# DeepMETv2/DeepMETv2

Measured on AMD Instinct MI355X. Metric: events/sec (4.5k PF cands, k=16), higher is better.
Workload: dtype f32

## Files before the change

deepmetv2_amd/build.py:

```python
from __future__ import annotations

import concurrent.futures as cf
import os
import shutil
import subprocess
import sys

PKG_DIR = os.path.dirname(os.path.abspath(__file__))
CSRC = os.path.join(PKG_DIR, "csrc")
OBJ_DIR = os.path.join(CSRC, "_obj")
LIB_PATH = os.path.join(PKG_DIR, "libdmet_hip.so")
SOURCES = ["knn.hip", "radius.hip", "edgeconv.hip", "edgemlp.hip", "misc.hip", "dense.hip", "encoder.hip", "norm.hip", "edgeconv_bwd.hip",
           "head.hip", "finalize.hip", "pool.hip",
           "edgemlp_f32.hip", "edgemlp_bf16.hip", "edgeconv_sum.hip", "gravnet.hip", "attention.hip", "fps.hip", "interpolate.hip",
           "pointnet.hip", "gat.hip", "segment.hip", "multi_aggr.hip", "weighted_sum.hip", "event_norm.hip", "select.hip"]
HEADERS = [os.path.join(CSRC, h) for h in ("common.h", "bn_affine.h", "knn_common.h", "knn_filter.h", "knn_key64.h", "knn_tile_schedule.h",
                                           "nls_body.h",
                                           "edgemlp_fused.h", "row_softmax.h")] + \
          [os.path.join(PKG_DIR, "..", "include", "dmet.h")]
ARCH = "gfx950"
CXXFLAGS = ["-O3", "-std=c++17", "-fPIC", f"--offload-arch={ARCH}", "-ffp-contract=off", "-Wall",
            "-Wno-unused-function", "-DNDEBUG"]


def _hipcc() -> str:
    exe = shutil.which("hipcc") or "/opt/rocm/bin/hipcc"
    if not os.path.exists(exe):
        raise RuntimeError("hipcc not found: cannot build libdmet_hip.so")
    return exe


def _stale(target: str, deps) -> bool:
    if not os.path.exists(target):
        return True
    t = os.path.getmtime(target)
    return any(os.path.getmtime(d) > t for d in deps if os.path.exists(d))


def _compile(src: str, force: bool) -> str:
    obj = os.path.join(OBJ_DIR, os.path.splitext(src)[0] + ".o")
    path = os.path.join(CSRC, src)
    if force or _stale(obj, [path] + HEADERS):
        cmd = [_hipcc()] + CXXFLAGS + ["-c", path, "-o", obj]
        subprocess.check_call(cmd)
    return obj


def build_hip(force: bool = False, verbose: bool = False) -> str:
    os.makedirs(OBJ_DIR, exist_ok=True)
    with cf.ThreadPoolExecutor(max_workers=min(4, len(SOURCES))) as ex:
        objs = list(ex.map(lambda s: _compile(s, force), SOURCES))
    if force or _stale(LIB_PATH, objs):
        cmd = [_hipcc(), "-shared", "-fPIC", f"--offload-arch={ARCH}", "-o", LIB_PATH] + objs
        if verbose:
            print(" ".join(cmd))
        subprocess.check_call(cmd)
    return LIB_PATH


if __name__ == "__main__":
    print(build_hip(force="--force" in sys.argv, verbose=True))
```

deepmetv2_amd/csrc/common.h:

```cpp
#pragma once
#include <hip/hip_runtime.h>
#include <stdint.h>
#include <stdio.h>
#include <stdlib.h>
#include <string.h>

#include <type_traits>

#include "../../include/dmet.h"

namespace dmet {

constexpr int kWave = 64;
constexpr int kNumXcd = 8;
constexpr float kKnnSentinel = 1e10f;

void set_error(const char *fmt, ...);
int hip_fail(hipError_t e, const char *what);

#define DMET_REQUIRE(cond, ...)                 \
    do {                                        \
        if (!(cond)) {                          \
            ::dmet::set_error(__VA_ARGS__);     \
            return -22;                         \
        }                                       \
    } while (0)

#define DMET_LAUNCH_CHECK(name)                                   \
    do {                                                          \
        hipError_t e__ = hipGetLastError();                       \
        if (e__ != hipSuccess) return ::dmet::hip_fail(e__, name); \
    } while (0)

static inline hipStream_t as_stream(dmet_stream_t s) { return reinterpret_cast<hipStream_t>(s); }

static inline bool env_is(const char *name, const char *value)
{
    const char *e = getenv(name);
    return e && strcmp(e, value) == 0;
}

static inline bool aligned16(const void *p) { return (reinterpret_cast<uintptr_t>(p) & 15u) == 0; }

__device__ __forceinline__ int find_event(const int64_t *__restrict__ ptr, int B, int64_t i)
{
    int lo = 0, hi = B;
    while (hi - lo > 1) {
        const int mid = (lo + hi) >> 1;
        if (ptr[mid] <= i) lo = mid; else hi = mid;
    }
    return lo;
}

__device__ __forceinline__ int xcd_swizzle(int bid, int nblk)
{
    const int q = nblk / kNumXcd, rm = nblk % kNumXcd;
    const int xcd = bid % kNumXcd, idx = bid / kNumXcd;
    const int base = (xcd < rm) ? xcd * (q + 1) : rm * (q + 1) + (xcd - rm) * q;
    return base + idx;
}

constexpr int kEcbPartialFloats = 2 * 1024 + 32;
constexpr int kEncPartialFloats = 3 * 1024 + 64;
constexpr int kHeadPartialFloats = 1024 + 64;
enum { kDeferEdgeConv = 0, kDeferEncoder = 1, kDeferHead = 2 };
struct DeferDesc {
    int kind;
    const float *partial;
    int64_t nparts;
    float *out[9];
};
bool defer_push(const DeferDesc &d);

__device__ __forceinline__ float wave_sum(float v)
{
#pragma unroll
    for (int off = 32; off > 0; off >>= 1) v += __shfl_xor(v, off, 64);
    return v;
}

template <int... Vs, typename F>
bool with_int(int v, F &&f)
{
    return ((v == Vs && (f(std::integral_constant<int, Vs>{}), true)) || ...);
}
template <typename F>
void with_flags(F &&f) { f(); }
template <typename F, typename... Rest>
void with_flags(F &&f, bool b, Rest... rest)
{
    if (b) with_flags([&](auto... c) { f(std::true_type{}, c...); }, rest...);
    else with_flags([&](auto... c) { f(std::false_type{}, c...); }, rest...);
}

}
```

deepmetv2_amd/csrc/encoder.hip:

```cpp
#include <stdlib.h>

#include "bn_affine.h"
#include "common.h"

namespace dmet {
namespace {

typedef float f32x16 __attribute__((ext_vector_type(16)));

#define ENC_PARAMS                                                                                                  \
    const float *__restrict__ Wc, const float *__restrict__ bc, const float *__restrict__ Wk,                      \
        const float *__restrict__ bk, const float *__restrict__ Wa, const float *__restrict__ ba,                  \
        const float *__restrict__ Echg, const float *__restrict__ Epdg, const float *__restrict__ Epv
#define ENC_ARGS Wc, bc, Wk, bk, Wa, ba, Echg, Epdg, Epv

__device__ __forceinline__ float elu(float z) { return z > 0.0f ? z : (__expf(z) - 1.0f); }

__device__ __forceinline__ void cat_indices(const int64_t *__restrict__ xcat, const float *__restrict__ row, int64_t i,
                                            int &ichg, int &ipdg, int &ipv)
{
    long long c = xcat ? xcat[i * 3 + 0] : (long long)row[8];
    const long long chg = xcat ? xcat[i * 3 + 1] : (long long)row[9];
    const long long pv = xcat ? xcat[i * 3 + 2] : (long long)row[10];
    c = c < 0 ? -c : c;
    const long long table[7] = {1, 2, 11, 13, 22, 130, 211};
#pragma unroll
    for (int t = 0; t < 7; ++t) c = (c == table[t]) ? (long long)t : c;
    ipdg = (int)min(max(c, 0ll), 6ll);
    ichg = (int)min(max(chg + 1, 0ll), 2ll);
    ipv = (int)min(max(pv, 0ll), 7ll);
}

__device__ __forceinline__ void encode_node(ENC_PARAMS, const float (&xc)[8], int ichg, int ipdg, int ipv,
                                            float (&cat24)[24], float (&z1)[16], float (&z2)[16], float (&joint)[32],
                                            float (&z3)[32])
{
#pragma unroll
    for (int e = 0; e < 8; ++e) {
        cat24[e] = Echg[ichg * 8 + e];
        cat24[8 + e] = Epdg[ipdg * 8 + e];
        cat24[16 + e] = Epv[ipv * 8 + e];
    }
#pragma unroll
    for (int o = 0; o < 16; ++o) {
        float a = bc[o];
#pragma unroll
        for (int f = 0; f < 8; ++f) a = __builtin_fmaf(Wc[o * 8 + f], xc[f], a);
        z1[o] = a;
        float b = bk[o];
#pragma unroll
        for (int f = 0; f < 24; ++f) b = __builtin_fmaf(Wk[o * 24 + f], cat24[f], b);
        z2[o] = b;
    }
#pragma unroll
    for (int o = 0; o < 16; ++o) { joint[o] = elu(z2[o]); joint[16 + o] = elu(z1[o]); }
#pragma unroll
    for (int o = 0; o < 32; ++o) {
        float a = ba[o];
#pragma unroll
        for (int f = 0; f < 32; ++f) a = __builtin_fmaf(Wa[o * 32 + f], joint[f], a);
        z3[o] = a;
    }
}

__global__ __launch_bounds__(256, 2) void encode_fwd_kernel(const float *__restrict__ x, int64_t x_stride,
                                                          const int64_t *__restrict__ xcat, int64_t N,
                                                          ENC_PARAMS, float *__restrict__ h)
{
    const int64_t i = (int64_t)blockIdx.x * blockDim.x + threadIdx.x;
    if (i >= N) return;
    const float *row = x + i * x_stride;
    float xc[8];
#pragma unroll
    for (int f = 0; f < 8; ++f) xc[f] = row[f];
    int ichg, ipdg, ipv;
    cat_indices(xcat, row, i, ichg, ipdg, ipv);
    float cat24[24], z1[16], z2[16], joint[32], z3[32];
    encode_node(ENC_ARGS, xc, ichg, ipdg, ipv, cat24, z1, z2, joint, z3);
    float4 *o = reinterpret_cast<float4 *>(h + i * 32);
#pragma unroll
    for (int c = 0; c < 8; ++c)
        o[c] = make_float4(elu(z3[4 * c]), elu(z3[4 * c + 1]), elu(z3[4 * c + 2]), elu(z3[4 * c + 3]));
}

__global__ __launch_bounds__(256) void encode_fwd_mfma_kernel(const float *__restrict__ x, int64_t x_stride,
                                                               const int64_t *__restrict__ xcat, int64_t N, ENC_PARAMS,
                                                               float *__restrict__ h)
{
    const int lane = threadIdx.x & 63, r = lane & 31, hh = lane >> 5;
    const int64_t wave = (int64_t)blockIdx.x * (blockDim.x >> 6) + __builtin_amdgcn_readfirstlane((int)(threadIdx.x >> 6));
    const int64_t nwaves = (int64_t)gridDim.x * (blockDim.x >> 6);
    const int64_t ntiles = (N + 31) / 32;
    float w12[16], w3[16], b12[16], b3[16];
#pragma unroll
    for (int s = 0; s < 16; ++s) {
        const int f = (s & 3) + 8 * (s >> 2) + 4 * hh;
        const float *src = r < 16 ? Wk + r * 24 + min(f, 23) : Wc + (r - 16) * 8 + max(f - 24, 0);
        const bool keep = r < 16 ? f < 24 : f >= 24;
        const float a = *src;
        w12[s] = keep ? a : 0.0f;
        w3[s] = Wa[r * 32 + f];
        const float *bsrc = f < 16 ? bk + f : bc + (f - 16);
        b12[s] = *bsrc;
        b3[s] = ba[f];
    }
    struct Raw { float c[4]; long long k0, k1, k2; };
    auto load_raw = [&](const int64_t tile, Raw &q) __attribute__((always_inline)) {
        const int64_t node = tile * 32 + r;
        const int64_t i = node < N ? node : N - 1;
        const float *row = x + i * x_stride;
#pragma unroll
        for (int u = 0; u < 4; ++u) q.c[u] = row[4 * hh + u];
        if (xcat) { q.k0 = xcat[i * 3 + 0]; q.k1 = xcat[i * 3 + 1]; q.k2 = xcat[i * 3 + 2]; }
        else { q.k0 = (long long)row[8]; q.k1 = (long long)row[9]; q.k2 = (long long)row[10]; }
    };
    auto load_tables = [&](const Raw &q, float (&in)[16]) __attribute__((always_inline)) {
        long long c = q.k0 < 0 ? -q.k0 : q.k0;
        const long long table[7] = {1, 2, 11, 13, 22, 130, 211};
#pragma unroll
        for (int t = 0; t < 7; ++t) c = (c == table[t]) ? (long long)t : c;
        const int ipdg = (int)min(max(c, 0ll), 6ll), ichg = (int)min(max(q.k1 + 1, 0ll), 2ll), ipv = (int)min(max(q.k2, 0ll), 7ll);
        const float4 e0 = *reinterpret_cast<const float4 *>(Echg + ichg * 8 + 4 * hh);
        const float4 e1 = *reinterpret_cast<const float4 *>(Epdg + ipdg * 8 + 4 * hh);
        const float4 e2 = *reinterpret_cast<const float4 *>(Epv + ipv * 8 + 4 * hh);
        in[0] = e0.x; in[1] = e0.y; in[2] = e0.z; in[3] = e0.w; in[4] = e1.x; in[5] = e1.y; in[6] = e1.z; in[7] = e1.w;
        in[8] = e2.x; in[9] = e2.y; in[10] = e2.z; in[11] = e2.w;
#pragma unroll
        for (int u = 0; u < 4; ++u) in[12 + u] = q.c[u];
    };
    Raw raw;
    float in[16], nxt[16];
    if (wave < ntiles) { load_raw(wave, raw); load_tables(raw, in); }
    if (wave + nwaves < ntiles) load_raw(wave + nwaves, raw);
    for (int64_t tile = wave; tile < ntiles; tile += nwaves) {
        const int64_t node = tile * 32 + r;
        if (tile + nwaves < ntiles) load_tables(raw, nxt);
        if (tile + 2 * nwaves < ntiles) load_raw(tile + 2 * nwaves, raw);
        f32x16 acc;
#pragma unroll
        for (int e = 0; e < 16; ++e) acc[e] = b12[e];
#pragma unroll
        for (int s = 0; s < 16; ++s) acc = __builtin_amdgcn_mfma_f32_32x32x2f32(w12[s], in[s], acc, 0, 0, 0);
        float joint[16];
#pragma unroll
        for (int e = 0; e < 16; ++e) joint[e] = elu(acc[e]);
#pragma unroll
        for (int e = 0; e < 16; ++e) acc[e] = b3[e];
#pragma unroll
        for (int s = 0; s < 16; ++s) acc = __builtin_amdgcn_mfma_f32_32x32x2f32(w3[s], joint[s], acc, 0, 0, 0);
        if (node < N) {
            float4 *o = reinterpret_cast<float4 *>(h + node * 32 + 4 * hh);
#pragma unroll
            for (int g = 0; g < 4; ++g)
                o[2 * g] = make_float4(elu(acc[4 * g]), elu(acc[4 * g + 1]), elu(acc[4 * g + 2]), elu(acc[4 * g + 3]));
        }
#pragma unroll
        for (int u = 0; u < 16; ++u) in[u] = nxt[u];
    }
}

constexpr int kEncTiles = 3;
constexpr int kEncBwdWaves = 4;
constexpr int kEncPartial = kEncTiles * 1024 + 64;

__device__ __forceinline__ void enc_wave_sync()
{
    __builtin_amdgcn_fence(__ATOMIC_RELEASE, "wavefront");
    __builtin_amdgcn_wave_barrier();
    __builtin_amdgcn_fence(__ATOMIC_ACQUIRE, "wavefront");
}

__device__ __forceinline__ void tile_mma(f32x16 &acc, const float *__restrict__ A, const float *__restrict__ Bm, int lane)
{
    const int c = lane & 31, hh = lane >> 5;
#pragma unroll 8
    for (int s = 0; s < 32; ++s) {
        const int node = 2 * s + hh;
        acc = __builtin_amdgcn_mfma_f32_32x32x2f32(A[node * 33 + c], Bm[node * 33 + c], acc, 0, 0, 0);
    }
}

__device__ __forceinline__ void tile_mma_onehot(f32x16 &acc, const int *__restrict__ packed, const float *__restrict__ Bm,
                                                int lane)
{
    const int c = lane & 31, hh = lane >> 5;
    int sh, mask, tgt;
    if (c < 3) { sh = 0; mask = 3; tgt = c; }
    else if (c < 10) { sh = 2; mask = 7; tgt = c - 3; }
    else if (c < 18) { sh = 5; mask = 7; tgt = c - 10; }
    else { sh = 0; mask = 0; tgt = 1; }
#pragma unroll 8
    for (int s = 0; s < 32; ++s) {
        const int node = 2 * s + hh;
        const float a = (((packed[node] >> sh) & mask) == tgt) ? 1.0f : 0.0f;
        acc = __builtin_amdgcn_mfma_f32_32x32x2f32(a, Bm[node * 33 + c], acc, 0, 0, 0);
    }
}

__device__ __forceinline__ float column_half_sum(const float *__restrict__ A, int lane)
{
    const int c = lane & 31, hh = lane >> 5;
    float s = 0.0f;
#pragma unroll 8
    for (int n = 0; n < 32; ++n) s += A[(hh * 32 + n) * 33 + c];
    return s;
}

__global__ __launch_bounds__(64 * kEncBwdWaves, 2) void encode_bwd_kernel(const float *__restrict__ x, int64_t x_stride,
                                                                          const int64_t *__restrict__ xcat, int64_t N,
                                                                          ENC_PARAMS, const float *__restrict__ gh,
                                                                          const float *__restrict__ hout,
                                                                          int64_t nodes_per_wave,
                                                                          float *__restrict__ partial)
{
    __shared__ float bufA[kEncBwdWaves][64 * 33];
    __shared__ float bufB[kEncBwdWaves][64 * 33];
    __shared__ int bufI[kEncBwdWaves][64];
    const int lane = threadIdx.x & 63, wv = __builtin_amdgcn_readfirstlane(threadIdx.x >> 6);
    float *A = bufA[wv], *Bm = bufB[wv];
    int *packed = bufI[wv];
    const int64_t wave = (int64_t)blockIdx.x * kEncBwdWaves + wv;
    const int64_t lo = wave * nodes_per_wave, hi = min(N, lo + nodes_per_wave);
    f32x16 acc[kEncTiles];
#pragma unroll
    for (int t = 0; t < kEncTiles; ++t)
#pragma unroll
        for (int e = 0; e < 16; ++e) acc[t][e] = 0.0f;
    float bias3 = 0.0f, bias21 = 0.0f;

    for (int64_t base = lo; base < hi; base += 64) {
        int zero = 0;
        asm volatile("" : "+s"(zero));
        const float *__restrict__ wc = Wc + zero, *__restrict__ wk = Wk + zero, *__restrict__ wa = Wa + zero,
                                  *__restrict__ pbc = bc + zero, *__restrict__ pbk = bk + zero;
        const int64_t i = base + lane;
        const bool live = i < hi;
        const int64_t ii = live ? i : (hi - 1);
        const float *row = x + ii * x_stride;
        float xc[8];
#pragma unroll
        for (int f = 0; f < 8; ++f) xc[f] = row[f];
        int ichg, ipdg, ipv;
        cat_indices(xcat, row, ii, ichg, ipdg, ipv);
        packed[lane] = ichg | (ipdg << 2) | (ipv << 5);
        float cat24[24], joint[32];
#pragma unroll
        for (int e = 0; e < 8; ++e) {
            cat24[e] = Echg[ichg * 8 + e];
            cat24[8 + e] = Epdg[ipdg * 8 + e];
            cat24[16 + e] = Epv[ipv * 8 + e];
        }
#pragma unroll
        for (int o = 0; o < 16; ++o) {
            float a = pbc[o];
#pragma unroll
            for (int f = 0; f < 8; ++f) a = __builtin_fmaf(wc[o * 8 + f], xc[f], a);
            joint[16 + o] = elu(a);
            float b = pbk[o];
#pragma unroll
            for (int f = 0; f < 24; ++f) b = __builtin_fmaf(wk[o * 24 + f], cat24[f], b);
            joint[o] = elu(b);
        }
        float gz[32];
        {
            const float4 *gp = reinterpret_cast<const float4 *>(gh + ii * 32);
            const float4 *hp = reinterpret_cast<const float4 *>(hout + ii * 32);
#pragma unroll
            for (int c4 = 0; c4 < 8; ++c4) {
                const float4 gv = gp[c4], hv = hp[c4];
                const float gg[4] = {gv.x, gv.y, gv.z, gv.w}, hh4[4] = {hv.x, hv.y, hv.z, hv.w};
#pragma unroll
                for (int u = 0; u < 4; ++u) {
                    const float d = hh4[u] > 0.0f ? 1.0f : (hh4[u] + 1.0f);
                    gz[4 * c4 + u] = live ? gg[u] * d : 0.0f;
                }
            }
        }
#pragma unroll
        for (int c = 0; c < 32; ++c) { A[lane * 33 + c] = gz[c]; Bm[lane * 33 + c] = joint[c]; }
        enc_wave_sync();
        tile_mma(acc[0], A, Bm, lane);
        bias3 += column_half_sum(A, lane);
        float gj[32];
#pragma unroll
        for (int f = 0; f < 32; ++f) gj[f] = 0.0f;
#pragma unroll
        for (int o = 0; o < 32; ++o)
#pragma unroll
            for (int f = 0; f < 32; ++f) gj[f] = __builtin_fmaf(wa[o * 32 + f], gz[o], gj[f]);
#pragma unroll
        for (int f = 0; f < 32; ++f) gj[f] *= joint[f] > 0.0f ? 1.0f : (joint[f] + 1.0f);
        enc_wave_sync();
#pragma unroll
        for (int c = 0; c < 32; ++c) {
            A[lane * 33 + c] = gj[c];
            Bm[lane * 33 + c] = (c < 24) ? cat24[c] : xc[c - 24];
        }
        enc_wave_sync();
        tile_mma(acc[1], A, Bm, lane);
        bias21 += column_half_sum(A, lane);
        float gc[24];
#pragma unroll
        for (int f = 0; f < 24; ++f) gc[f] = 0.0f;
#pragma unroll
        for (int o = 0; o < 16; ++o)
#pragma unroll
            for (int f = 0; f < 24; ++f) gc[f] = __builtin_fmaf(wk[o * 24 + f], gj[o], gc[f]);
        enc_wave_sync();
#pragma unroll
        for (int c = 0; c < 32; ++c) Bm[lane * 33 + c] = (c < 24) ? gc[c < 24 ? c : 0] : 0.0f;
        enc_wave_sync();
        tile_mma_onehot(acc[2], packed, Bm, lane);
        enc_wave_sync();
    }
    const int c = lane & 31, hh = lane >> 5;
    __syncthreads();
#pragma unroll
    for (int e = 0; e < 16; ++e) {
        const int r = (e & 3) + 8 * (e >> 2) + 4 * hh;
        A[r * 32 + c] = acc[0][e];
        A[1024 + r * 32 + c] = acc[2][e];
        Bm[r * 32 + c] = acc[1][e];
    }
    const float b3 = bias3 + __shfl_xor(bias3, 32), b21 = bias21 + __shfl_xor(bias21, 32);
    if (hh == 0) { Bm[1024 + c] = b3; Bm[1024 + 32 + c] = b21; }
    __syncthreads();
    float *out = partial + (int64_t)blockIdx.x * kEncPartial;
    for (int i = threadIdx.x; i < kEncPartial; i += 64 * kEncBwdWaves) {
        const float *src = i < 1024 ? &bufA[0][i] : i < 2048 ? &bufB[0][i - 1024] : i < 3072 ? &bufA[0][i - 1024]
                                                                                              : &bufB[0][i - 2048];
        float t = src[0];
#pragma unroll
        for (int w = 1; w < kEncBwdWaves; ++w) t += src[w * 64 * 33];
        out[i] = t;
    }
}

__device__ __forceinline__ void enc_lds_sync()
{
    asm volatile("s_waitcnt lgkmcnt(0)" ::: "memory");
    __builtin_amdgcn_wave_barrier();
}

__device__ __forceinline__ void tile_mma32(f32x16 &acc, const float *__restrict__ A, const float *__restrict__ Bm, int lane)
{
    const int c = lane & 31, hh = lane >> 5;
#pragma unroll 8
    for (int s = 0; s < 16; ++s) {
        const int node = 2 * s + hh;
        acc = __builtin_amdgcn_mfma_f32_32x32x2f32(A[node * 33 + c], Bm[node * 33 + c], acc, 0, 0, 0);
    }
}

__device__ __forceinline__ void tile_mma_onehot32(f32x16 &acc, const int *__restrict__ packed, const float *__restrict__ Bm,
                                                  int lane)
{
    const int c = lane & 31, hh = lane >> 5;
    int sh, mask, tgt;
    if (c < 3) { sh = 0; mask = 3; tgt = c; }
    else if (c < 10) { sh = 2; mask = 7; tgt = c - 3; }
    else if (c < 18) { sh = 5; mask = 7; tgt = c - 10; }
    else { sh = 0; mask = 0; tgt = 1; }
#pragma unroll 8
    for (int s = 0; s < 16; ++s) {
        const int node = 2 * s + hh;
        const float a = (((packed[node] >> sh) & mask) == tgt) ? 1.0f : 0.0f;
        acc = __builtin_amdgcn_mfma_f32_32x32x2f32(a, Bm[node * 33 + c], acc, 0, 0, 0);
    }
}

__device__ __forceinline__ float column_half_sum32(const float *__restrict__ A, int lane)
{
    const int c = lane & 31, hh = lane >> 5;
    float s = 0.0f;
#pragma unroll 8
    for (int n = 0; n < 16; ++n) s += A[(hh * 16 + n) * 33 + c];
    return s;
}

struct EncBnBwd {
    const float *gamma, *mean, *invstd, *mean_g, *mean_gx;
};

template <bool BNB = false>
__global__ __launch_bounds__(64 * kEncBwdWaves, 2) void encode_bwd_mfma_kernel(const float *__restrict__ x, int64_t x_stride,
                                                                               const int64_t *__restrict__ xcat, int64_t N,
                                                                               ENC_PARAMS, const float *__restrict__ gh,
                                                                               const float *__restrict__ hout,
                                                                               int64_t ,
                                                                               float *__restrict__ partial,
                                                                               EncBnBwd bnb = EncBnBwd{})
{
    __shared__ float bufA[kEncBwdWaves][64 * 33];
    __shared__ float bufB[kEncBwdWaves][64 * 33];
    __shared__ int bufI[kEncBwdWaves][64];
    const int lane = threadIdx.x & 63, wv = __builtin_amdgcn_readfirstlane(threadIdx.x >> 6);
    const int r = lane & 31, hh = lane >> 5;
    float *A = bufA[wv], *Bm = bufB[wv];
    int *packed = bufI[wv];
    const int64_t wave = (int64_t)blockIdx.x * kEncBwdWaves + wv, nwaves = (int64_t)gridDim.x * kEncBwdWaves;
    const int64_t ntiles = (N + 31) / 32, hi = N;
    float w12[16], w3t[16], w12t[16], b12[16];
#pragma unroll
    for (int s = 0; s < 16; ++s) {
        const int f = (s & 3) + 8 * (s >> 2) + 4 * hh;
        {
            const float *src = r < 16 ? Wk + r * 24 + min(f, 23) : Wc + (r - 16) * 8 + max(f - 24, 0);
            const bool keep = r < 16 ? f < 24 : f >= 24;
            const float a = *src;
            w12[s] = keep ? a : 0.0f;
        }
        w3t[s] = Wa[f * 32 + r];
        {
            const float *src = f < 16 ? Wk + f * 24 + min(r, 23) : Wc + (f - 16) * 8 + max(r - 24, 0);
            const bool keep = f < 16 ? r < 24 : r >= 24;
            const float a = *src;
            w12t[s] = keep ? a : 0.0f;
        }
        const float *bsrc = f < 16 ? bk + f : bc + (f - 16);
        b12[s] = *bsrc;
    }
    f32x16 acc[kEncTiles];
#pragma unroll
    for (int t = 0; t < kEncTiles; ++t)
#pragma unroll
        for (int e = 0; e < 16; ++e) acc[t][e] = 0.0f;
    float bias3 = 0.0f, bias21 = 0.0f;

    struct Raw { float c[4]; long long k0, k1, k2; };
    auto load_raw = [&](const int64_t tile, Raw &q) __attribute__((always_inline)) {
        const int64_t nd = tile * 32 + r;
        const int64_t i = nd < N ? nd : N - 1;
        const float *row = x + i * x_stride;
#pragma unroll
        for (int u = 0; u < 4; ++u) q.c[u] = row[4 * hh + u];
        if (xcat) { q.k0 = xcat[i * 3 + 0]; q.k1 = xcat[i * 3 + 1]; q.k2 = xcat[i * 3 + 2]; }
        else { q.k0 = (long long)row[8]; q.k1 = (long long)row[9]; q.k2 = (long long)row[10]; }
    };
    auto load_tables = [&](const Raw &q, float (&in)[16], int &pk) __attribute__((always_inline)) {
        long long c = q.k0 < 0 ? -q.k0 : q.k0;
        const long long table[7] = {1, 2, 11, 13, 22, 130, 211};
#pragma unroll
        for (int t = 0; t < 7; ++t) c = (c == table[t]) ? (long long)t : c;
        const int ipdg = (int)min(max(c, 0ll), 6ll), ichg = (int)min(max(q.k1 + 1, 0ll), 2ll), ipv = (int)min(max(q.k2, 0ll), 7ll);
        pk = ichg | (ipdg << 2) | (ipv << 5);
        const float4 e0 = *reinterpret_cast<const float4 *>(Echg + ichg * 8 + 4 * hh);
        const float4 e1 = *reinterpret_cast<const float4 *>(Epdg + ipdg * 8 + 4 * hh);
        const float4 e2 = *reinterpret_cast<const float4 *>(Epv + ipv * 8 + 4 * hh);
        in[0] = e0.x; in[1] = e0.y; in[2] = e0.z; in[3] = e0.w; in[4] = e1.x; in[5] = e1.y; in[6] = e1.z; in[7] = e1.w;
        in[8] = e2.x; in[9] = e2.y; in[10] = e2.z; in[11] = e2.w;
#pragma unroll
        for (int u = 0; u < 4; ++u) in[12 + u] = q.c[u];
    };
    Raw raw;
    float in[16], nxt[16];
    int pk = 0, pk_nxt = 0;
    if (wave < ntiles) { load_raw(wave, raw); load_tables(raw, in, pk); }
    if (wave + nwaves < ntiles) load_raw(wave + nwaves, raw);
    for (int64_t tile = wave; tile < ntiles; tile += nwaves) {
        const int64_t node = tile * 32 + r;
        const bool live = node < hi;
        const int64_t ii = live ? node : (hi - 1);
        if (tile + nwaves < ntiles) load_tables(raw, nxt, pk_nxt);
        if (tile + 2 * nwaves < ntiles) load_raw(tile + 2 * nwaves, raw);
        if (hh == 0) packed[r] = pk;
        float gz[16];
        {
            const float4 *gp = reinterpret_cast<const float4 *>(gh + ii * 32 + 4 * hh);
            const float4 *hp = reinterpret_cast<const float4 *>(hout + ii * 32 + 4 * hh);
#pragma unroll
            for (int g = 0; g < 4; ++g) {
                float4 gv = gp[2 * g];
                const float4 hv = hp[2 * g];
                if constexpr (BNB) {
                    const int c0 = 8 * g + 4 * hh;
                    const float4 ga = *reinterpret_cast<const float4 *>(bnb.gamma + c0), mu = *reinterpret_cast<const float4 *>(bnb.mean + c0);
                    const float4 is = *reinterpret_cast<const float4 *>(bnb.invstd + c0), mg = *reinterpret_cast<const float4 *>(bnb.mean_g + c0);
                    const float4 mx = *reinterpret_cast<const float4 *>(bnb.mean_gx + c0);
                    gv = bn_bwd4(gv, hv, ga, mu, is, mg, mx);
                }
                const float gg[4] = {gv.x, gv.y, gv.z, gv.w}, hh4[4] = {hv.x, hv.y, hv.z, hv.w};
#pragma unroll
                for (int u = 0; u < 4; ++u) {
                    const float d = hh4[u] > 0.0f ? 1.0f : (hh4[u] + 1.0f);
                    gz[4 * g + u] = live ? gg[u] * d : 0.0f;
                }
            }
        }
        f32x16 c1;
#pragma unroll
        for (int e = 0; e < 16; ++e) c1[e] = b12[e];
#pragma unroll
        for (int s = 0; s < 16; ++s) c1 = __builtin_amdgcn_mfma_f32_32x32x2f32(w12[s], in[s], c1, 0, 0, 0);
        float joint[16];
#pragma unroll
        for (int e = 0; e < 16; ++e) joint[e] = elu(c1[e]);
#pragma unroll
        for (int e = 0; e < 16; ++e) {
            const int ch = (e & 3) + 8 * (e >> 2) + 4 * hh;
            A[r * 33 + ch] = gz[e];
            Bm[r * 33 + ch] = joint[e];
        }
        enc_lds_sync();
        tile_mma32(acc[0], A, Bm, lane);
        bias3 += column_half_sum32(A, lane);
        f32x16 c2;
#pragma unroll
        for (int e = 0; e < 16; ++e) c2[e] = 0.0f;
#pragma unroll
        for (int s = 0; s < 16; ++s) c2 = __builtin_amdgcn_mfma_f32_32x32x2f32(w3t[s], gz[s], c2, 0, 0, 0);
        float gj[16];
#pragma unroll
        for (int e = 0; e < 16; ++e) gj[e] = c2[e] * (joint[e] > 0.0f ? 1.0f : (joint[e] + 1.0f));
        enc_lds_sync();
#pragma unroll
        for (int e = 0; e < 16; ++e) {
            const int ch = (e & 3) + 8 * (e >> 2) + 4 * hh;
            A[r * 33 + ch] = gj[e];
            Bm[r * 33 + ch] = in[e];
        }
        enc_lds_sync();
        tile_mma32(acc[1], A, Bm, lane);
        bias21 += column_half_sum32(A, lane);
        f32x16 c3;
#pragma unroll
        for (int e = 0; e < 16; ++e) c3[e] = 0.0f;
#pragma unroll
        for (int s = 0; s < 16; ++s) c3 = __builtin_amdgcn_mfma_f32_32x32x2f32(w12t[s], gj[s], c3, 0, 0, 0);
        enc_lds_sync();
#pragma unroll
        for (int e = 0; e < 16; ++e) {
            const int ch = (e & 3) + 8 * (e >> 2) + 4 * hh;
            Bm[r * 33 + ch] = ch < 24 ? c3[e] : 0.0f;
        }
        enc_lds_sync();
        tile_mma_onehot32(acc[2], packed, Bm, lane);
        enc_lds_sync();
#pragma unroll
        for (int u = 0; u < 16; ++u) in[u] = nxt[u];
        pk = pk_nxt;
    }
    const int c = lane & 31;
    __syncthreads();
#pragma unroll
    for (int e = 0; e < 16; ++e) {
        const int rr = (e & 3) + 8 * (e >> 2) + 4 * hh;
        A[rr * 32 + c] = acc[0][e];
        A[1024 + rr * 32 + c] = acc[2][e];
        Bm[rr * 32 + c] = acc[1][e];
    }
    const float b3 = bias3 + __shfl_xor(bias3, 32), b21 = bias21 + __shfl_xor(bias21, 32);
    if (hh == 0) { Bm[1024 + c] = b3; Bm[1024 + 32 + c] = b21; }
    __syncthreads();
    float *out = partial + (int64_t)blockIdx.x * kEncPartial;
    for (int i = threadIdx.x; i < kEncPartial; i += 64 * kEncBwdWaves) {
        const float *src = i < 1024 ? &bufA[0][i] : i < 2048 ? &bufB[0][i - 1024] : i < 3072 ? &bufA[0][i - 1024]
                                                                                              : &bufB[0][i - 2048];
        float t = src[0];
#pragma unroll
        for (int w = 1; w < kEncBwdWaves; ++w) t += src[w * 64 * 33];
        out[i] = t;
    }
}

struct EncGrads {
    float *Wc, *bc, *Wk, *bk, *Wa, *ba, *Echg, *Epdg, *Epv;
};

__global__ __launch_bounds__(1024) void encode_bwd_finalize_kernel(const float *__restrict__ partial, int64_t nwaves,
                                                                    EncGrads g)
{
    __shared__ float red[32][33];
    const int e = threadIdx.x & 31, grp = threadIdx.x >> 5;
    const int idx = blockIdx.x * 32 + e;
    float s = 0.0f;
#pragma unroll 8
    for (int64_t w = grp; w < nwaves; w += 32) s += partial[w * kEncPartial + idx];
    red[grp][e] = s;
    __syncthreads();
    if (grp != 0) return;
    s = 0.0f;
#pragma unroll
    for (int q = 0; q < 32; ++q) s += red[q][e];
    const int t = idx / 1024, r = (idx % 1024) / 32, c = idx % 32;
    if (t == 0) g.Wa[r * 32 + c] = s;
    else if (t == 1) {
        if (r < 16 && c < 24) g.Wk[r * 24 + c] = s;
        else if (r >= 16 && c >= 24) g.Wc[(r - 16) * 8 + (c - 24)] = s;
    } else if (t == 2) {
        if (r < 3 && c < 8) g.Echg[r * 8 + c] = s;
        else if (r >= 3 && r < 10 && c >= 8 && c < 16) g.Epdg[(r - 3) * 8 + (c - 8)] = s;
        else if (r >= 10 && r < 18 && c >= 16 && c < 24) g.Epv[(r - 10) * 8 + (c - 16)] = s;
    } else if (r == 0) g.ba[c] = s;
    else if (c < 16) g.bk[c] = s;
    else g.bc[c - 16] = s;
}

inline int64_t enc_nodes_per_wave(int64_t N, int64_t *nwaves)
{
    const int64_t target_waves = 2048;
    int64_t npw = (N + target_waves - 1) / target_waves;
#ifdef DMET_ENC_NPW_UP
    npw = (npw + 63) / 64 * 64;
#else
    npw = npw / 64 * 64;
#endif
    if (npw < 64) npw = 64;
    int64_t nw = (N + npw - 1) / npw;
    nw = (nw + kEncBwdWaves - 1) / kEncBwdWaves * kEncBwdWaves;
    *nwaves = nw;
    return npw;
}

thread_local EncBnBwd g_enc_bnb{nullptr, nullptr, nullptr, nullptr, nullptr};
thread_local bool g_enc_bnb_done = false;

}
}

using namespace dmet;

extern "C" int dmet_encode_fwd_f32(const float *x, int64_t x_stride, const int64_t *xcat, int64_t N, const float *Wc, const float *bc,
                                   const float *Wk, const float *bk, const float *Wa, const float *ba,
                                   const float *Echg, const float *Epdg, const float *Epv, float *h,
                                   dmet_stream_t stream)
{
    DMET_REQUIRE(N >= 0 && x_stride >= 8, "dmet_encode_fwd_f32: bad sizes");
    if (N == 0) return 0;
    DMET_REQUIRE(x && Wc && bc && Wk && bk && Wa && ba && Echg && Epdg && Epv && h, "dmet_encode_fwd_f32: null pointer");
    DMET_REQUIRE(xcat || x_stride >= 11, "dmet_encode_fwd_f32: x_cat == NULL needs rows of at least 11 columns (x_stride=%lld)", (long long)x_stride);
    DMET_REQUIRE(aligned16(h), "dmet_encode_fwd_f32: h must be 16-B aligned");
    const int64_t blocks = (N + 255) / 256;
    DMET_REQUIRE(blocks < (1ll << 31), "dmet_encode_fwd_f32: too many nodes");
    const int form = env_is("DMET_ENCODER_FWD", "valu") ? 0 : 1;
    if (form == 1 && aligned16(Echg) && aligned16(Epdg) && aligned16(Epv)) {
        const int64_t tiles = (N + 31) / 32;
        int64_t grid = (tiles + 3) / 4;
        int gmax = 512;
        if (const char *e = getenv("DMET_ENC_GRID")) { gmax = atoi(e); if (gmax < 1) gmax = 512; }
        if (grid > gmax) grid = gmax;
        hipLaunchKernelGGL(encode_fwd_mfma_kernel, dim3((unsigned)grid), dim3(256), 0, as_stream(stream), x, x_stride, xcat, N,
                           ENC_ARGS, h);
        DMET_LAUNCH_CHECK("encode_fwd_mfma_kernel");
        return 0;
    }
    hipLaunchKernelGGL(encode_fwd_kernel, dim3((unsigned)blocks), dim3(256), 0, as_stream(stream), x, x_stride, xcat, N, ENC_ARGS, h);
    DMET_LAUNCH_CHECK("encode_fwd_kernel");
    return 0;
}

extern "C" size_t dmet_encode_bwd_workspace_bytes(int64_t N)
{
    if (N <= 0) return 0;
    int64_t nw;
    (void)enc_nodes_per_wave(N, &nw);
    return sizeof(float) * (size_t)nw * kEncPartial + 512;
}

extern "C" int dmet_encode_bwd_f32(const float *x, int64_t x_stride, const int64_t *xcat, int64_t N, const float *Wc, const float *bc,
                                   const float *Wk, const float *bk, const float *Wa, const float *ba,
                                   const float *Echg, const float *Epdg, const float *Epv, const float *h,
                                   const float *g_h, float *gWc, float *gbc, float *gWk, float *gbk, float *gWa,
                                   float *gba, float *gEchg, float *gEpdg, float *gEpv, void *ws, size_t ws_bytes,
                                   dmet_stream_t stream)
{
    DMET_REQUIRE(N > 0 && x_stride >= 8, "dmet_encode_bwd_f32: bad sizes");
    DMET_REQUIRE((xcat || x_stride >= 11) && x && Wc && bc && Wk && bk && Wa && ba && Echg && Epdg && Epv && h && g_h && gWc && gbc && gWk && gbk &&
                     gWa && gba && gEchg && gEpdg && gEpv && ws,
                 "dmet_encode_bwd_f32: null pointer");
    DMET_REQUIRE(ws_bytes >= dmet_encode_bwd_workspace_bytes(N), "dmet_encode_bwd_f32: workspace too small");
    DMET_REQUIRE(aligned16(h) && aligned16(g_h), "dmet_encode_bwd_f32: h / g_h must be 16-B aligned");
    int64_t nw;
    const int64_t npw = enc_nodes_per_wave(N, &nw);
    float *partial = reinterpret_cast<float *>((reinterpret_cast<uintptr_t>(ws) + 255u) & ~(uintptr_t)255u);
    hipStream_t st = as_stream(stream);
    const int form = env_is("DMET_ENCODER_BWD", "valu") ? 0 : 1;
    int64_t nparts = nw / kEncBwdWaves;
    if (form == 1 && aligned16(Echg) && aligned16(Epdg) && aligned16(Epv) && aligned16(g_h) && aligned16(h)) {
        const int64_t tiles = (N + 31) / 32;
        int64_t grid = (tiles + kEncBwdWaves - 1) / kEncBwdWaves;
        if (grid > 512) grid = 512;
        if (grid > nparts) grid = nparts;
        nparts = grid;
        if (g_enc_bnb.gamma)
            hipLaunchKernelGGL(encode_bwd_mfma_kernel<true>, dim3((unsigned)grid), dim3(64 * kEncBwdWaves), 0, st, x, x_stride, xcat,
                               N, ENC_ARGS, g_h, h, npw, partial, g_enc_bnb);
        else
            hipLaunchKernelGGL(encode_bwd_mfma_kernel<false>, dim3((unsigned)grid), dim3(64 * kEncBwdWaves), 0, st, x, x_stride,
                               xcat, N, ENC_ARGS, g_h, h, npw, partial, EncBnBwd{});
        g_enc_bnb_done = g_enc_bnb.gamma != nullptr;
    } else {
        hipLaunchKernelGGL(encode_bwd_kernel, dim3((unsigned)(nw / kEncBwdWaves)), dim3(64 * kEncBwdWaves), 0, st, x, x_stride,
                           xcat, N, ENC_ARGS, g_h, h, npw, partial);
    }
    DMET_LAUNCH_CHECK("encode_bwd_kernel");
    EncGrads gr{gWc, gbc, gWk, gbk, gWa, gba, gEchg, gEpdg, gEpv};
    static_assert(kEncPartial % 32 == 0, "finalize blocks own 32 elements");
    static_assert(kEncPartial == kEncPartialFloats, "csrc/finalize.hip sums the same partial layout");
    if (defer_push(DeferDesc{kDeferEncoder, partial, nparts, {gWc, gbc, gWk, gbk, gWa, gba, gEchg, gEpdg, gEpv}})) return 0;
    hipLaunchKernelGGL(encode_bwd_finalize_kernel, dim3(kEncPartial / 32), dim3(1024), 0, st, partial, nparts, gr);
    DMET_LAUNCH_CHECK("encode_bwd_finalize_kernel");
    return 0;
}

extern "C" int dmet_encode_bn_bwd_f32(const float *x, int64_t x_stride, const int64_t *xcat, int64_t N, const float *Wc,
                                      const float *bc, const float *Wk, const float *bk, const float *Wa, const float *ba,
                                      const float *Echg, const float *Epdg, const float *Epv, const float *h,
                                      const float *g_y, const float *bn_gamma, const float *bn_mean, const float *bn_invstd,
                                      const float *bn_mean_g, const float *bn_mean_gx, float *gWc, float *gbc, float *gWk,
                                      float *gbk, float *gWa, float *gba, float *gEchg, float *gEpdg, float *gEpv,
                                      int *fused, void *ws, size_t ws_bytes, dmet_stream_t stream)
{
    DMET_REQUIRE(fused, "dmet_encode_bn_bwd_f32: fused is null");
    *fused = 0;
    DMET_REQUIRE(bn_gamma && bn_mean && bn_invstd && bn_mean_g && bn_mean_gx, "dmet_encode_bn_bwd_f32: null pointer");
    const bool ok = !env_is("DMET_ENCODER_BWD", "valu") && N > 0 && aligned16(Echg) && aligned16(Epdg) && aligned16(Epv) && aligned16(g_y) &&
                    aligned16(h) && aligned16(bn_gamma) && aligned16(bn_mean) && aligned16(bn_invstd) && aligned16(bn_mean_g) &&
                    aligned16(bn_mean_gx);
    if (!ok) return 0;
    g_enc_bnb = EncBnBwd{bn_gamma, bn_mean, bn_invstd, bn_mean_g, bn_mean_gx};
    g_enc_bnb_done = false;
    const int rc = dmet_encode_bwd_f32(x, x_stride, xcat, N, Wc, bc, Wk, bk, Wa, ba, Echg, Epdg, Epv, h, g_y, gWc, gbc, gWk, gbk, gWa,
                                       gba, gEchg, gEpdg, gEpv, ws, ws_bytes, stream);
    const bool done = g_enc_bnb_done;
    g_enc_bnb = EncBnBwd{nullptr, nullptr, nullptr, nullptr, nullptr};
    g_enc_bnb_done = false;
    if (rc == 0 && !done) {
        set_error("dmet_encode_bn_bwd_f32: the matrix-core backward it was checked for did not run");
        return -22;
    }
    *fused = rc == 0 ? 1 : 0;
    return rc;
}
```

Baseline: 52900.

## Batch LDS loads before MFMA chains and overlap row loads with first GEMM

Moves the tile MFMA helpers into a shared header, where they now issue batches of eight LDS loads, fenced by scheduler barriers, before eight back-to-back MFMAs. In the encoder backward kernel, gradient and activation rows are fetched with inline-asm global loads that are issued before the first MFMA chain and waited on afterwards, so global latency overlaps matrix work. Batch-norm backward parameters are staged once per block into shared memory instead of being reloaded from global memory for every tile. The changes add register pressure and fix the instruction schedule by hand, which may fight the compiler's own scheduling.

```diff
diff --git a/deepmetv2_amd/build.py b/deepmetv2_amd/build.py
--- a/deepmetv2_amd/build.py
+++ b/deepmetv2_amd/build.py
@@ -15,7 +15,7 @@
            "edgemlp_f32.hip", "edgemlp_bf16.hip", "edgeconv_sum.hip", "gravnet.hip", "attention.hip", "fps.hip", "interpolate.hip",
            "pointnet.hip", "gat.hip", "segment.hip", "multi_aggr.hip", "weighted_sum.hip", "event_norm.hip", "select.hip"]
 HEADERS = [os.path.join(CSRC, h) for h in ("common.h", "bn_affine.h", "knn_common.h", "knn_filter.h", "knn_key64.h", "knn_tile_schedule.h",
-                                           "nls_body.h",
+                                           "nls_body.h", "mfma_tile.h",
                                            "edgemlp_fused.h", "row_softmax.h")] + \
           [os.path.join(PKG_DIR, "..", "include", "dmet.h")]
 ARCH = "gfx950"
diff --git a/deepmetv2_amd/csrc/common.h b/deepmetv2_amd/csrc/common.h
--- a/deepmetv2_amd/csrc/common.h
+++ b/deepmetv2_amd/csrc/common.h
@@ -79,6 +79,12 @@
     return v;
 }
 
+__device__ __forceinline__ void lds_wave_sync()
+{
+    asm volatile("s_waitcnt lgkmcnt(0)" ::: "memory");
+    __builtin_amdgcn_wave_barrier();
+}
+
 template <int... Vs, typename F>
 bool with_int(int v, F &&f)
 {
diff --git a/deepmetv2_amd/csrc/encoder.hip b/deepmetv2_amd/csrc/encoder.hip
--- a/deepmetv2_amd/csrc/encoder.hip
+++ b/deepmetv2_amd/csrc/encoder.hip
@@ -2,6 +2,7 @@
 
 #include "bn_affine.h"
 #include "common.h"
+#include "mfma_tile.h"
 
 namespace dmet {
 namespace {
@@ -336,51 +337,18 @@
     }
 }
 
-__device__ __forceinline__ void enc_lds_sync()
-{
-    asm volatile("s_waitcnt lgkmcnt(0)" ::: "memory");
-    __builtin_amdgcn_wave_barrier();
-}
-
-__device__ __forceinline__ void tile_mma32(f32x16 &acc, const float *__restrict__ A, const float *__restrict__ Bm, int lane)
-{
-    const int c = lane & 31, hh = lane >> 5;
-#pragma unroll 8
-    for (int s = 0; s < 16; ++s) {
-        const int node = 2 * s + hh;
-        acc = __builtin_amdgcn_mfma_f32_32x32x2f32(A[node * 33 + c], Bm[node * 33 + c], acc, 0, 0, 0);
-    }
-}
-
-__device__ __forceinline__ void tile_mma_onehot32(f32x16 &acc, const int *__restrict__ packed, const float *__restrict__ Bm,
-                                                  int lane)
-{
-    const int c = lane & 31, hh = lane >> 5;
-    int sh, mask, tgt;
-    if (c < 3) { sh = 0; mask = 3; tgt = c; }
-    else if (c < 10) { sh = 2; mask = 7; tgt = c - 3; }
-    else if (c < 18) { sh = 5; mask = 7; tgt = c - 10; }
-    else { sh = 0; mask = 0; tgt = 1; }
-#pragma unroll 8
-    for (int s = 0; s < 16; ++s) {
-        const int node = 2 * s + hh;
-        const float a = (((packed[node] >> sh) & mask) == tgt) ? 1.0f : 0.0f;
-        acc = __builtin_amdgcn_mfma_f32_32x32x2f32(a, Bm[node * 33 + c], acc, 0, 0, 0);
-    }
-}
-
-__device__ __forceinline__ float column_half_sum32(const float *__restrict__ A, int lane)
-{
-    const int c = lane & 31, hh = lane >> 5;
-    float s = 0.0f;
-#pragma unroll 8
-    for (int n = 0; n < 16; ++n) s += A[(hh * 16 + n) * 33 + c];
-    return s;
-}
-
 struct EncBnBwd {
     const float *gamma, *mean, *invstd, *mean_g, *mean_gx;
 };
+
+typedef float enc_f32x4 __attribute__((ext_vector_type(4)));
+#define ENC_LOAD_ROW(v0, v1, v2, v3, p)                                                                              \
+    asm volatile("global_load_dwordx4 %0, %4, off\n\tglobal_load_dwordx4 %1, %4, off offset:32\n\t"                 \
+                 "global_load_dwordx4 %2, %4, off offset:64\n\tglobal_load_dwordx4 %3, %4, off offset:96"            \
+                 : "=&v"(v0), "=&v"(v1), "=&v"(v2), "=&v"(v3) : "v"(p) : "memory")
+#define ENC_ROWS_WAIT(acc, a0, a1, a2, a3, b0, b1, b2, b3)                                                           \
+    asm volatile("s_waitcnt vmcnt(0)"                                                                                \
+                 : "+v"(acc), "+v"(a0), "+v"(a1), "+v"(a2), "+v"(a3), "+v"(b0), "+v"(b1), "+v"(b2), "+v"(b3) :: "memory")
 
 template <bool BNB = false>
 __global__ __launch_bounds__(64 * kEncBwdWaves, 2) void encode_bwd_mfma_kernel(const float *__restrict__ x, int64_t x_stride,
@@ -394,10 +362,21 @@
     __shared__ float bufA[kEncBwdWaves][64 * 33];
     __shared__ float bufB[kEncBwdWaves][64 * 33];
     __shared__ int bufI[kEncBwdWaves][64];
+    __shared__ __attribute__((aligned(16))) float sBn[BNB ? 5 : 1][32];
     const int lane = threadIdx.x & 63, wv = __builtin_amdgcn_readfirstlane(threadIdx.x >> 6);
     const int r = lane & 31, hh = lane >> 5;
     float *A = bufA[wv], *Bm = bufB[wv];
     int *packed = bufI[wv];
+    if constexpr (BNB) {
+        if (threadIdx.x < 160) {
+            const float *src[5] = {bnb.gamma, bnb.mean, bnb.invstd, bnb.mean_g, bnb.mean_gx};
+            const float *p = src[0];
+#pragma unroll
+            for (int q = 1; q < 5; ++q) p = (int)(threadIdx.x >> 5) == q ? src[q] : p;
+            sBn[threadIdx.x >> 5][threadIdx.x & 31] = p[threadIdx.x & 31];
+        }
+        __syncthreads();
+    }
     const int64_t wave = (int64_t)blockIdx.x * kEncBwdWaves + wv, nwaves = (int64_t)gridDim.x * kEncBwdWaves;
     const int64_t ntiles = (N + 31) / 32, hi = N;
     float w12[16], w3t[16], w12t[16], b12[16];
@@ -464,19 +443,30 @@
         if (tile + nwaves < ntiles) load_tables(raw, nxt, pk_nxt);
         if (tile + 2 * nwaves < ntiles) load_raw(tile + 2 * nwaves, raw);
         if (hh == 0) packed[r] = pk;
+        enc_f32x4 gv0, gv1, gv2, gv3, hv0, hv1, hv2, hv3;
+        {
+            const float *gp = gh + ii * 32 + 4 * hh, *hp = hout + ii * 32 + 4 * hh;
+            ENC_LOAD_ROW(gv0, gv1, gv2, gv3, gp);
+            ENC_LOAD_ROW(hv0, hv1, hv2, hv3, hp);
+        }
+        f32x16 c1;
+#pragma unroll
+        for (int e = 0; e < 16; ++e) c1[e] = b12[e];
+#pragma unroll
+        for (int s = 0; s < 16; ++s) c1 = __builtin_amdgcn_mfma_f32_32x32x2f32(w12[s], in[s], c1, 0, 0, 0);
+        ENC_ROWS_WAIT(c1, gv0, gv1, gv2, gv3, hv0, hv1, hv2, hv3);
+        const enc_f32x4 gvv[4] = {gv0, gv1, gv2, gv3}, hvv[4] = {hv0, hv1, hv2, hv3};
         float gz[16];
         {
-            const float4 *gp = reinterpret_cast<const float4 *>(gh + ii * 32 + 4 * hh);
-            const float4 *hp = reinterpret_cast<const float4 *>(hout + ii * 32 + 4 * hh);
 #pragma unroll
             for (int g = 0; g < 4; ++g) {
-                float4 gv = gp[2 * g];
-                const float4 hv = hp[2 * g];
+                float4 gv = make_float4(gvv[g].x, gvv[g].y, gvv[g].z, gvv[g].w);
+                const float4 hv = make_float4(hvv[g].x, hvv[g].y, hvv[g].z, hvv[g].w);
                 if constexpr (BNB) {
                     const int c0 = 8 * g + 4 * hh;
-                    const float4 ga = *reinterpret_cast<const float4 *>(bnb.gamma + c0), mu = *reinterpret_cast<const float4 *>(bnb.mean + c0);
-                    const float4 is = *reinterpret_cast<const float4 *>(bnb.invstd + c0), mg = *reinterpret_cast<const float4 *>(bnb.mean_g + c0);
-                    const float4 mx = *reinterpret_cast<const float4 *>(bnb.mean_gx + c0);
+                    const float4 ga = *reinterpret_cast<const float4 *>(&sBn[0][c0]), mu = *reinterpret_cast<const float4 *>(&sBn[1][c0]);
+                    const float4 is = *reinterpret_cast<const float4 *>(&sBn[2][c0]), mg = *reinterpret_cast<const float4 *>(&sBn[3][c0]);
+                    const float4 mx = *reinterpret_cast<const float4 *>(&sBn[4][c0]);
                     gv = bn_bwd4(gv, hv, ga, mu, is, mg, mx);
                 }
                 const float gg[4] = {gv.x, gv.y, gv.z, gv.w}, hh4[4] = {hv.x, hv.y, hv.z, hv.w};
@@ -487,11 +477,6 @@
                 }
             }
         }
-        f32x16 c1;
-#pragma unroll
-        for (int e = 0; e < 16; ++e) c1[e] = b12[e];
-#pragma unroll
-        for (int s = 0; s < 16; ++s) c1 = __builtin_amdgcn_mfma_f32_32x32x2f32(w12[s], in[s], c1, 0, 0, 0);
         float joint[16];
 #pragma unroll
         for (int e = 0; e < 16; ++e) joint[e] = elu(c1[e]);
@@ -501,9 +486,9 @@
             A[r * 33 + ch] = gz[e];
             Bm[r * 33 + ch] = joint[e];
         }
-        enc_lds_sync();
-        tile_mma32(acc[0], A, Bm, lane);
-        bias3 += column_half_sum32(A, lane);
+        lds_wave_sync();
+        tile_mma32<33>(acc[0], A, Bm, lane);
+        bias3 += column_half_sum32<33>(A, lane);
         f32x16 c2;
 #pragma unroll
         for (int e = 0; e < 16; ++e) c2[e] = 0.0f;
@@ -512,30 +497,30 @@
         float gj[16];
 #pragma unroll
         for (int e = 0; e < 16; ++e) gj[e] = c2[e] * (joint[e] > 0.0f ? 1.0f : (joint[e] + 1.0f));
-        enc_lds_sync();
+        lds_wave_sync();
 #pragma unroll
         for (int e = 0; e < 16; ++e) {
             const int ch = (e & 3) + 8 * (e >> 2) + 4 * hh;
             A[r * 33 + ch] = gj[e];
             Bm[r * 33 + ch] = in[e];
         }
-        enc_lds_sync();
-        tile_mma32(acc[1], A, Bm, lane);
-        bias21 += column_half_sum32(A, lane);
+        lds_wave_sync();
+        tile_mma32<33>(acc[1], A, Bm, lane);
+        bias21 += column_half_sum32<33>(A, lane);
         f32x16 c3;
 #pragma unroll
         for (int e = 0; e < 16; ++e) c3[e] = 0.0f;
 #pragma unroll
         for (int s = 0; s < 16; ++s) c3 = __builtin_amdgcn_mfma_f32_32x32x2f32(w12t[s], gj[s], c3, 0, 0, 0);
-        enc_lds_sync();
+        lds_wave_sync();
 #pragma unroll
         for (int e = 0; e < 16; ++e) {
             const int ch = (e & 3) + 8 * (e >> 2) + 4 * hh;
             Bm[r * 33 + ch] = ch < 24 ? c3[e] : 0.0f;
         }
-        enc_lds_sync();
-        tile_mma_onehot32(acc[2], packed, Bm, lane);
-        enc_lds_sync();
+        lds_wave_sync();
+        tile_mma_onehot32<33>(acc[2], packed, Bm, lane);
+        lds_wave_sync();
 #pragma unroll
         for (int u = 0; u < 16; ++u) in[u] = nxt[u];
         pk = pk_nxt;
diff --git a/deepmetv2_amd/csrc/mfma_tile.h b/deepmetv2_amd/csrc/mfma_tile.h
--- /dev/null
+++ b/deepmetv2_amd/csrc/mfma_tile.h
@@ -0,0 +1,70 @@
+#pragma once
+#include <hip/hip_runtime.h>
+
+namespace dmet {
+
+typedef float mfma_f32x16 __attribute__((ext_vector_type(16)));
+constexpr int kMfmaTileBatch = 8;
+
+template <int STRIDE>
+__device__ __forceinline__ void tile_mma32(mfma_f32x16 &acc, const float *__restrict__ A, const float *__restrict__ Bm, int lane)
+{
+    const int c = lane & 31, hh = lane >> 5;
+#pragma unroll 1
+    for (int h = 0; h < 16; h += kMfmaTileBatch) {
+        float a[kMfmaTileBatch], b[kMfmaTileBatch];
+#pragma unroll
+        for (int s = 0; s < kMfmaTileBatch; ++s) {
+            a[s] = A[(2 * (h + s) + hh) * STRIDE + c];
+            b[s] = Bm[(2 * (h + s) + hh) * STRIDE + c];
+        }
+        __builtin_amdgcn_sched_barrier(0);
+#pragma unroll
+        for (int s = 0; s < kMfmaTileBatch; ++s) acc = __builtin_amdgcn_mfma_f32_32x32x2f32(a[s], b[s], acc, 0, 0, 0);
+        __builtin_amdgcn_sched_barrier(0);
+    }
+}
+
+template <int STRIDE>
+__device__ __forceinline__ void tile_mma_onehot32(mfma_f32x16 &acc, const int *__restrict__ packed, const float *__restrict__ Bm,
+                                                  int lane)
+{
+    const int c = lane & 31, hh = lane >> 5;
+    int sh, mask, tgt;
+    if (c < 3) { sh = 0; mask = 3; tgt = c; }
+    else if (c < 10) { sh = 2; mask = 7; tgt = c - 3; }
+    else if (c < 18) { sh = 5; mask = 7; tgt = c - 10; }
+    else { sh = 0; mask = 0; tgt = 1; }
+#pragma unroll 1
+    for (int h = 0; h < 16; h += kMfmaTileBatch) {
+        int p[kMfmaTileBatch];
+        float b[kMfmaTileBatch];
+#pragma unroll
+        for (int s = 0; s < kMfmaTileBatch; ++s) {
+            p[s] = packed[2 * (h + s) + hh];
+            b[s] = Bm[(2 * (h + s) + hh) * STRIDE + c];
+        }
+        __builtin_amdgcn_sched_barrier(0);
+#pragma unroll
+        for (int s = 0; s < kMfmaTileBatch; ++s) {
+            const float a = (((p[s] >> sh) & mask) == tgt) ? 1.0f : 0.0f;
+            acc = __builtin_amdgcn_mfma_f32_32x32x2f32(a, b[s], acc, 0, 0, 0);
+        }
+        __builtin_amdgcn_sched_barrier(0);
+    }
+}
+
+template <int STRIDE>
+__device__ __forceinline__ float column_half_sum32(const float *__restrict__ A, int lane)
+{
+    const int c = lane & 31, hh = lane >> 5;
+    float v[16];
+#pragma unroll
+    for (int n = 0; n < 16; ++n) v[n] = A[(hh * 16 + n) * STRIDE + c];
+    float s = 0.0f;
+#pragma unroll
+    for (int n = 0; n < 16; ++n) s += v[n];
+    return s;
+}
+
+}
```

Result: no change. 52960, median of 2 (+0.1%).
